# mdnunez/bayesflow_nddms

Measured on AMD Instinct MI355X. Metric: simulated DDM trials/sec at n_trials=300 dt=0.001 (basic_ddm_dc, max_steps=4000), higher is better.
Workload: dtype f32

## Files before the change

### bayesflow_nddms_amd/_lib.py

```python
import ctypes
import os

from .build import SO_PATH

NDDM_OK, NDDM_ERR_NULL, NDDM_ERR_SHAPE, NDDM_ERR_PARAM, NDDM_ERR_HIP, NDDM_ERR_NO_DEVICE = range(6)
GAUSS_EXACT, GAUSS_FAST, BRIDGE, GAUSS_PACKED, STATE_F64 = 0, 1, 2, 4, 8
QUANTILE_CONDITIONAL = 1
HMC_SIGMA_FIXED = 1
ABI_VERSION = 4

_lib = None


class NddmLibraryError(ImportError):
    pass


def _declare(L):
    c = ctypes
    fp, vp = c.c_void_p, c.c_void_p
    L.nddm_abi_version.restype = c.c_int
    L.nddm_last_error.restype = c.c_char_p
    L.nddm_device_count.argtypes = [c.POINTER(c.c_int)]
    L.nddm_set_device.argtypes = [c.c_int]
    L.nddm_summary_k.restype = c.c_int
    L.nddm_model_nparams.argtypes = [c.c_int]
    L.nddm_set_tuning.argtypes = [c.c_int] * 6
    L.nddm_set_debug_trace.argtypes = [c.c_void_p, c.c_int, c.c_int]
    L.nddm_set_ordering.argtypes = [c.c_int]
    L.nddm_debug_set_slot_limit.argtypes = [c.c_int]
    L.nddm_debug_last_launch.argtypes = [c.POINTER(c.c_int32)]
    common = [c.c_int64, c.c_int32, c.c_float, c.c_int32, c.c_uint64, c.c_uint64, c.c_uint32]
    for name in ("nddm_basic_ddm_dc_simulate", "nddm_single_trial_simulate", "nddm_single_trial_alt_simulate"):
        getattr(L, name).argtypes = [fp] + common + [fp, fp, vp]
    L.nddm_alpha_not_scaled_simulate.argtypes = [fp] + common + [c.c_float, c.c_int32, fp, fp, fp, vp]
    L.nddm_explicit_boundary_simulate.argtypes = [fp, fp] + common + [fp, fp, vp]
    L.nddm_simulratcliff.argtypes = [fp, c.c_int64, c.c_int32, c.c_uint64, c.c_uint64, c.c_uint32, c.c_float, c.c_int32, fp, fp, fp, vp]
    L.nddm_wiener_log_likelihood.argtypes = [c.c_int32, fp, c.c_int64, c.c_int64, fp, c.c_int32, c.c_uint32, fp, fp, vp]
    L.nddm_wiener_cdf.argtypes = [c.c_int32, fp, c.c_int64, c.c_int64, fp, c.c_int32, c.c_uint32, fp, fp, vp]
    L.nddm_wiener_log_likelihood_grad.argtypes = [c.c_int32, fp, c.c_int64, c.c_int64, fp, c.c_int32, c.c_uint32, fp, fp, vp]
    L.nddm_wiener_marginal_log_likelihood.argtypes = [c.c_int32, fp, c.c_int64, c.c_int64, fp, c.c_int32, c.c_float, c.c_uint32, fp, fp, vp]
    L.nddm_wiener_marginal_log_likelihood_grad.argtypes = [c.c_int32, fp, c.c_int64, c.c_int64, fp, c.c_int32, c.c_float, c.c_uint32, fp, fp, vp]
    L.nddm_wiener_hmc.argtypes = [c.c_int32, fp, c.c_int64, c.c_int32, c.c_int64, c.c_int64, fp, fp, c.c_int32, c.c_int32, c.c_int32, c.c_int32,
                                  c.c_uint32, c.c_uint64, c.c_uint64, c.c_uint64, c.c_uint32, fp, fp, fp, fp, fp, vp]
    L.nddm_wiener_hmc_joint.argtypes = [c.c_int32, fp, c.c_int64, c.c_int32, c.c_int64, c.c_int64, fp, fp, fp, fp, fp, c.c_int32, c.c_int32, c.c_int32,
                                        c.c_int32, c.c_uint32, c.c_uint64, c.c_uint64, c.c_uint64, c.c_uint32, fp, fp, fp, fp, fp, fp, fp, vp]
    L.nddm_wiener_quantile.argtypes = [c.c_int32, fp, c.c_int64, c.c_int64, fp, c.c_int32, c.c_uint32, fp, vp]
    L.nddm_simulate.argtypes = [c.c_int32, fp, fp] + common + [c.c_float, c.c_int32, fp, fp, fp, vp]
    L.nddm_simulate_indirect.argtypes = [c.c_int32, fp, fp] + common[:-1] + [fp, c.c_uint32, c.c_float, c.c_int32, fp, fp, fp, vp]
    L.nddm_simulate_codes.argtypes = [c.c_int32, fp] + common[:-1] + [fp, c.c_uint32, fp, fp, fp, vp]
    L.nddm_decode_codes.argtypes = [c.c_int32, fp, fp, c.c_int64, c.c_int32, c.c_float, fp, vp]
    L.nddm_draw_prior.argtypes = [c.c_int32, c.c_int64, c.c_uint64, c.c_uint64, c.c_float, fp, vp]
    L.nddm_draw_prior_indirect.argtypes = [c.c_int32, c.c_int64, c.c_uint64, c.c_uint64, fp, c.c_float, fp, vp]
    L.nddm_graph_arena_create.argtypes = [c.POINTER(c.c_uint64)]
    L.nddm_graph_arena_bind.argtypes = [c.c_uint64, c.POINTER(c.c_uint64)]
    L.nddm_graph_arena_info.argtypes = [c.c_uint64, c.POINTER(c.c_uint64), c.POINTER(c.c_int32)]
    L.nddm_graph_arena_release.argtypes = [c.c_uint64]
    L.nddm_source_hash.restype = c.c_char_p
    L.nddm_build_info.restype = c.c_char_p
    L.nddm_debug_normals.argtypes = [fp, c.c_int64, c.c_uint32, c.c_uint32, c.c_uint32, fp, vp]
    for name in EXPORTS:
        if name not in ("nddm_last_error", "nddm_source_hash", "nddm_build_info"):
            getattr(L, name).restype = c.c_int


EXPORTS = [
    "nddm_abi_version", "nddm_last_error", "nddm_device_count", "nddm_set_device", "nddm_summary_k",
    "nddm_model_nparams", "nddm_basic_ddm_dc_simulate", "nddm_single_trial_simulate",
    "nddm_single_trial_alt_simulate", "nddm_alpha_not_scaled_simulate", "nddm_explicit_boundary_simulate",
    "nddm_simulate", "nddm_draw_prior", "nddm_debug_normals", "nddm_set_tuning", "nddm_set_debug_trace", "nddm_set_ordering",
    "nddm_release_graph_memory", "nddm_debug_set_slot_limit", "nddm_debug_last_launch",
    "nddm_simulate_indirect", "nddm_draw_prior_indirect", "nddm_source_hash", "nddm_simulate_codes", "nddm_decode_codes",
    "nddm_graph_arena_create", "nddm_graph_arena_bind", "nddm_graph_arena_info", "nddm_graph_arena_release", "nddm_build_info",
    "nddm_simulratcliff", "nddm_wiener_log_likelihood", "nddm_wiener_cdf", "nddm_wiener_quantile",
    "nddm_wiener_log_likelihood_grad", "nddm_wiener_marginal_log_likelihood", "nddm_wiener_marginal_log_likelihood_grad",
    "nddm_wiener_hmc", "nddm_wiener_hmc_joint",
]


def lib():
    global _lib
    if _lib is None:
        from .build import build_hip, embedded_hash, is_stale, source_hash
        override = bool(os.environ.get("NDDM_HIP_LIB"))
        if is_stale():
            try:
                build_hip()
            except Exception as e:
                why = "is missing" if not os.path.exists(SO_PATH) else \
                    f"was built from other sources (library {embedded_hash()}, tree {source_hash()})"
                raise NddmLibraryError(
                    f"{SO_PATH} {why} and could not be rebuilt ({e!r}): build it with "
                    "`python -c 'import __graft_entry__ as g; g.build()'` (hipcc --offload-arch=gfx950).  "
                    "There is no CPU fallback.") from e
        if not os.path.exists(SO_PATH):
            raise NddmLibraryError(f"{SO_PATH} does not exist (NDDM_HIP_LIB points to a missing file?).  There is no CPU fallback.")
        import torch
        try:
            L = ctypes.CDLL(SO_PATH)
        except OSError as e:
            raise NddmLibraryError(f"cannot load {SO_PATH}: {e}") from e
        missing = [name for name in EXPORTS if not hasattr(L, name)]
        if missing:
            raise NddmLibraryError(f"{SO_PATH} does not export {missing}: it is older than this binding -- rebuild it "
                                   "(`python -c 'import __graft_entry__ as g; g.build()'`)")
        _declare(L)
        if L.nddm_abi_version() != ABI_VERSION:
            raise NddmLibraryError(f"ABI mismatch: library {L.nddm_abi_version()} != binding {ABI_VERSION} "
                                   "(the random stream differs between ABI versions): rebuild the library")
# ... 15 lines not shown
```

### bayesflow_nddms_amd/build.py

```python
import hashlib
import os
import re
import shutil
import subprocess

_HERE = os.path.dirname(os.path.abspath(__file__))
SO_PATH = os.environ.get("NDDM_HIP_LIB") or os.path.join(_HERE, "libnddm_hip.so")
SOURCES = [os.path.join(_HERE, "csrc", "nddm_kernels.hip")]
HEADERS = [os.path.join(_HERE, "csrc", "nddm_rng.h"), os.path.join(_HERE, "csrc", "nddm_sim.h"),
           os.path.join(_HERE, "csrc", "nddm_prepass.h"), os.path.join(_HERE, "csrc", "nddm_ratcliff.h"),
           os.path.join(_HERE, "csrc", "nddm_wiener.h"), os.path.join(_HERE, "csrc", "nddm_wiener_cdf.h"),
           os.path.join(_HERE, "csrc", "nddm_wiener_quantile.h"), os.path.join(_HERE, "csrc", "nddm_wiener_grad.h"),
           os.path.join(_HERE, "csrc", "nddm_wiener_marginal.h"), os.path.join(_HERE, "csrc", "nddm_wiener_marginal_grad.h"),
           os.path.join(_HERE, "csrc", "nddm_wiener_hmc.h"),
           os.path.join(_HERE, "csrc", "nddm_wiener_hmc_joint.h"),
           os.path.join(os.path.dirname(_HERE), "include", "nddm.h")]
HIPCC_FLAGS = ["-O3", "-ffp-contract=off", "--offload-arch=gfx950", "-fPIC", "-shared", "-std=c++17"]


def _hipcc():
    exe = shutil.which("hipcc") or "/opt/rocm/bin/hipcc"
    if not os.path.exists(exe):
        raise RuntimeError("hipcc not found: the HIP extension cannot be built")
    return exe


def source_hash():
    h = hashlib.sha256()
    for p in SOURCES + HEADERS:
        h.update(os.path.basename(p).encode() + b"\0")
        with open(p, "rb") as f:
            h.update(f.read())
        h.update(b"\0")
    h.update(" ".join(HIPCC_FLAGS).encode())
    return h.hexdigest()


def embedded_hash(path=None):
    path = path or SO_PATH
    try:
        with open(path, "rb") as f:
            m = re.search(rb"NDDM_SRC_HASH=([0-9a-f]{64})", f.read())
# ... 89 lines not shown
```

### bayesflow_nddms_amd/csrc/nddm_kernels.hip

```cpp
#include <hip/hip_runtime.h>
#include <math.h>
#include <stdint.h>
#include <stdio.h>
#include <stdlib.h>
#include <string.h>

#include <mutex>
#include <thread>

#include "../../include/nddm.h"
#include "nddm_prepass.h"
#include "nddm_ratcliff.h"
#include "nddm_rng.h"
#include "nddm_sim.h"
#include "nddm_wiener.h"
#include "nddm_wiener_cdf.h"
#include "nddm_wiener_grad.h"
#include "nddm_wiener_hmc.h"
#include "nddm_wiener_hmc_joint.h"
#include "nddm_wiener_marginal.h"
#include "nddm_wiener_marginal_grad.h"
#include "nddm_wiener_quantile.h"

namespace nddm {

static thread_local char g_err[512] = "";

static int fail(int code, const char *fmt, const char *detail = "")
{
    snprintf(g_err, sizeof g_err, fmt, detail);
    return code;
}

static int round_up_pow2(int v) { int p = 1; while (p < v) p <<= 1; return p; }

static int check_stream(hipStream_t st)
{
    int sdev = -1, cur = -1;
    const hipError_t e = hipStreamGetDevice(st, &sdev);
    if (e != hipSuccess) {
        (void)hipGetLastError();
        return fail(NDDM_ERR_HIP, "`stream` is not a live stream of this process's HIP runtime (destroyed, or created by another copy "
                                  "of the runtime): %s", hipGetErrorString(e));
    }
    if (hipGetDevice(&cur) == hipSuccess && st != nullptr && st != hipStreamPerThread && sdev != cur)
        return fail(NDDM_ERR_PARAM, "`stream` belongs to another device than the current one (nddm_set_device / hipSetDevice)%s");
    return NDDM_OK;
}

struct Tuning { int sets_per_chunk, ring, refill_thresh, variant, grid_waves, tile_trials, no_order; };
struct LastLaunch { int grid_waves, vkeys, ring, tile_trials, tiles_per_set, sets_per_chunk, refill_thresh, lds_bytes; };
static thread_local LastLaunch g_last = {0, 0, 0, 0, 0, 0, 0, 0};
static std::mutex g_mu;
static Tuning g_tuning = {0, 0, 0, 0, 0, 0, 0};
static unsigned long long *g_dbg = nullptr;
static int g_dbg_waves = 0, g_dbg_chunks = 0;

constexpr int MAX_DEVICES = 64;
struct DeviceInfo { int cus = 0; double clock_hz = 0.0; };
static DeviceInfo g_dev[MAX_DEVICES];

static bool device_info(int dev, DeviceInfo *out)
{
    std::lock_guard<std::mutex> lock(g_mu);
    if (g_dev[dev].cus == 0) {
        hipDeviceProp_t prop;
        if (hipGetDeviceProperties(&prop, dev) != hipSuccess) return false;
        g_dev[dev].cus = prop.multiProcessorCount > 0 ? prop.multiProcessorCount : 1;
        g_dev[dev].clock_hz = prop.clockRate > 0 ? (double)prop.clockRate * 1e3 : 2.4e9;
    }
    *out = g_dev[dev];
    return true;
}

constexpr size_t SLOT_QUEUE_BYTES = 256, SLOT_SCRATCH = 1u << 20;
constexpr int MAX_SLOTS = 256;
struct LaunchSlot {
    char *base = nullptr;
    hipEvent_t done = nullptr;
    hipStream_t stream = nullptr;
    bool busy = false;
    bool fresh = true;
};
static LaunchSlot *g_slots[MAX_DEVICES][MAX_SLOTS];
static int g_nslots[MAX_DEVICES];
static int g_slot_limit = MAX_SLOTS;

// ... 119 lines not shown
    *err = malloc_relaxed(&p, bytes);
    if (*err != hipSuccess) return nullptr;
    std::lock_guard<std::mutex> lock(g_mu);
    GraphArena *a = find_arena_locked(g_cur_arena);
    if (!a) a = &g_ownerless;
    a->list = new GraphAlloc{p, dev, bytes, a->list};
    return static_cast<char *>(p);
}

__global__ void zero_words_kernel(unsigned int *ws) { ws[threadIdx.x] = 0u; }

template <typename K>
static int resident_waves(K kernel, size_t lds_bytes, int cus)
{
    int per_cu = 0;
    if (hipOccupancyMaxActiveBlocksPerMultiprocessor(&per_cu, kernel, WAVE, lds_bytes) != hipSuccess || per_cu < 1)
        per_cu = 8;
    if (per_cu > 32) per_cu = 32;
    {
        const size_t granules = (lds_bytes + 1279) / 1280;
        const int by_lds = granules ? (int)((160u * 1024u) / (granules * 1280)) : 32;
        if (per_cu > by_lds) per_cu = by_lds;
    }
    hipFuncAttributes fa;
    if (hipFuncGetAttributes(&fa, reinterpret_cast<const void *>(kernel)) == hipSuccess && fa.numRegs > 0) {
        int per_simd = 512 / (((fa.numRegs + 7) / 8) * 8);
        if (per_simd < 1) per_simd = 1;
        if (per_cu > 4 * per_simd) per_cu = 4 * per_simd;
    }
    if (per_cu < 1) per_cu = 1;
    return cus * per_cu;
}

template <int MODEL, bool BRIDGE, bool SMALL, bool PACKED, bool VKEYS, bool CODES = false, bool F64 = false>
static void launch_variant(const SimArgs &A, bool fast, bool cap4, size_t lds_bytes, int n_chunks, int cus, int grid_override,
                           bool grid_forced, hipStream_t st)
{
    const dim3 block(WAVE);
#define NDDM_LAUNCH(KERNEL)                                                                    \
    do {                                                                                       \
        int waves = resident_waves(KERNEL, lds_bytes, cus);                                    \
        if (grid_override > 0 && (grid_override < waves || grid_forced)) waves = grid_override;\
        if (waves > n_chunks) waves = n_chunks;                                                \
        g_last.grid_waves = waves; g_last.vkeys = VKEYS ? 1 : 0;                               \
        hipLaunchKernelGGL(KERNEL, dim3(waves), block, lds_bytes, st, A);                      \
    } while (0)
    if (fast && cap4)       NDDM_LAUNCH((sim_kernel<MODEL, true, true, BRIDGE, SMALL, PACKED, VKEYS, CODES, F64>));
    else if (fast)          NDDM_LAUNCH((sim_kernel<MODEL, true, false, BRIDGE, SMALL, PACKED, VKEYS, CODES, F64>));
    else if (cap4)          NDDM_LAUNCH((sim_kernel<MODEL, false, true, BRIDGE, SMALL, PACKED, VKEYS, CODES, F64>));
    else                    NDDM_LAUNCH((sim_kernel<MODEL, false, false, BRIDGE, SMALL, PACKED, VKEYS, CODES, F64>));
#undef NDDM_LAUNCH
}

template <int MODEL, bool BRIDGE>
static int launch_model(const SimArgs &A, bool fast, bool packed, bool vkeys, bool f64, size_t lds_bytes, int n_chunks, int cus,
                        int grid_override, bool grid_forced, hipStream_t st)
{
    const bool cap4 = (A.max_k % ((packed || BRIDGE) ? 8 : 4)) == 0;
    const bool small = A.res16 == 2;
    constexpr bool HAS_VKEYS = !BRIDGE && (MODEL == NDDM_BASIC_DDM_DC || MODEL == NDDM_ALPHA_NOT_SCALED || MODEL == NDDM_EXPLICIT_BOUNDARY);
#define NDDM_ARGS A, fast, cap4, lds_bytes, n_chunks, cus, grid_override, grid_forced, st
    constexpr bool HAS_CODES = !BRIDGE && (MODEL == NDDM_BASIC_DDM_DC || MODEL == NDDM_ALPHA_NOT_SCALED);
    constexpr bool HAS_F64 = !BRIDGE && (MODEL == NDDM_BASIC_DDM_DC || MODEL == NDDM_SINGLE_TRIAL);
    if (f64) {
        if constexpr (HAS_F64) {
            if (small) launch_variant<MODEL, false, true, false, false, false, true>(NDDM_ARGS);
            else launch_variant<MODEL, false, false, false, false, false, true>(NDDM_ARGS);
        }
    }
    else if (A.out_codes) {
        if constexpr (HAS_CODES) launch_variant<MODEL, false, true, false, false, true>(NDDM_ARGS);
    }
    else if constexpr (BRIDGE) launch_variant<MODEL, true, false, false, false>(NDDM_ARGS);
    else if (!small && !packed) launch_variant<MODEL, false, false, false, false>(NDDM_ARGS);
    else if constexpr (HAS_VKEYS) {
        if (packed && vkeys) launch_variant<MODEL, false, true, true, true>(NDDM_ARGS);
        else if (packed) launch_variant<MODEL, false, true, true, false>(NDDM_ARGS);
        else if (vkeys) launch_variant<MODEL, false, true, false, true>(NDDM_ARGS);
        else launch_variant<MODEL, false, true, false, false>(NDDM_ARGS);
    } else {
        if (packed) launch_variant<MODEL, false, true, true, false>(NDDM_ARGS);
        else launch_variant<MODEL, false, true, false, false>(NDDM_ARGS);
    }
#undef NDDM_ARGS
    const hipError_t e = hipGetLastError();
    if (e != hipSuccess) return fail(NDDM_ERR_HIP, "kernel launch failed: %s", hipGetErrorString(e));
    return NDDM_OK;
}

static int simulate(int model, const float *params, const float *bounds, int64_t B, int32_t n_trials, float dt,
                    int32_t max_steps, uint64_t seed, uint64_t set_offset, const uint64_t *set_offset_dev, uint32_t flags,
                    float ext_sigma, int32_t ext_mode, float *out_trials, float *out_summary, float *out_ext, void *stream,
                    uint16_t *out_codes = nullptr)
{
// ... 180 lines not shown
    }
    int rc = NDDM_OK;
    A.partials = want_partials ? reinterpret_cast<unsigned long long *>(scratch + order_bytes) : nullptr;
    {
        const int threads = 256;
        long long blocks = (B + threads - 1) / threads;
        hipError_t e = hipSuccess;
        const int rec_mode = (fast ? 1 : 0) | (f64 ? 2 : 0);
        if (want_order) {
            int *order_ws = reinterpret_cast<int *>(scratch);
            uint32_t *recs = reinterpret_cast<uint32_t *>(order_ws + 64);
            if (blocks > 2048) blocks = 2048;
            hipLaunchKernelGGL(zero_words_kernel, dim3(1), dim3(64), 0, st, reinterpret_cast<unsigned int *>(order_ws));
            hipLaunchKernelGGL(order_hist_kernel, dim3((unsigned)blocks), dim3(threads), 0, st, model, params, P, (int)B, dt,
                               (int)max_steps, order_ws);
            hipLaunchKernelGGL(order_scatter_kernel, dim3((unsigned)blocks), dim3(threads), 0, st, model, rec_mode, params, P,
                               (int)B, dt, A.sqrt_dt, (int)max_steps, (unsigned long long)set_offset,
                               reinterpret_cast<const unsigned long long *>(set_offset_dev), order_ws, recs);
            A.recs = recs;
        } else {
            uint32_t *recs = reinterpret_cast<uint32_t *>(scratch);
            hipLaunchKernelGGL(prep_kernel, dim3((unsigned)blocks), dim3(threads), 0, st, model, rec_mode, params, P, (int)B, dt,
                               A.sqrt_dt, (unsigned long long)set_offset, reinterpret_cast<const unsigned long long *>(set_offset_dev), recs);
            A.recs = recs;
        }
        e = hipGetLastError();
        if (e != hipSuccess) rc = fail(NDDM_ERR_HIP, "pre-pass (hand-out records): %s", hipGetErrorString(e));
    }
    if (rc == NDDM_OK) {
        const int gw = plan_waves < 8ll * simds || tun.grid_waves > 0 ? (int)plan_waves : 0;
        bool vkeys = plan_waves < 8ll * simds || n_chunks < 8ll * simds || est_blocks < 2.0e4 * (double)simds;
        if (tun.variant % 3 == 1) vkeys = false;
        else if (tun.variant % 3 == 2) vkeys = true;
        g_last.ring = ring; g_last.tile_trials = tile_n; g_last.tiles_per_set = tiles; g_last.sets_per_chunk = spc;
        g_last.refill_thresh = A.refill_thresh; g_last.lds_bytes = (int)lds;
        switch (model) {
        case NDDM_BASIC_DDM_DC: rc = launch_model<NDDM_BASIC_DDM_DC, false>(A, fast, packed, vkeys, f64, lds, (int)n_chunks, di.cus, gw, tun.grid_waves > 0, st); break;
        case NDDM_SINGLE_TRIAL: rc = launch_model<NDDM_SINGLE_TRIAL, false>(A, fast, packed, vkeys, f64, lds, (int)n_chunks, di.cus, gw, tun.grid_waves > 0, st); break;
        case NDDM_SINGLE_TRIAL_ALT: rc = launch_model<NDDM_SINGLE_TRIAL_ALT, false>(A, fast, packed, vkeys, f64, lds, (int)n_chunks, di.cus, gw, tun.grid_waves > 0, st); break;
        case NDDM_ALPHA_NOT_SCALED:
            rc = bridge ? launch_model<NDDM_ALPHA_NOT_SCALED, true>(A, fast, packed, vkeys, f64, lds, (int)n_chunks, di.cus, gw, tun.grid_waves > 0, st)
                        : launch_model<NDDM_ALPHA_NOT_SCALED, false>(A, fast, packed, vkeys, f64, lds, (int)n_chunks, di.cus, gw, tun.grid_waves > 0, st);
            break;
        default: rc = launch_model<NDDM_EXPLICIT_BOUNDARY, false>(A, fast, packed, vkeys, f64, lds, (int)n_chunks, di.cus, gw, tun.grid_waves > 0, st); break;
        }
    }
    if (rc == NDDM_OK && A.partials) {
        const int tau_idx = model == NDDM_EXPLICIT_BOUNDARY ? 2 : 3;
        const int threads = 256;
        hipLaunchKernelGGL(combine_partials_kernel, dim3((unsigned)((B + threads - 1) / threads)), dim3(threads), 0, st,
                           A.partials, pw, params, P, tau_idx, (long long)B, tiles, n_trials, A.tscale, out_summary);
        const hipError_t e = hipGetLastError();
        if (e != hipSuccess) rc = fail(NDDM_ERR_HIP, "combine kernel launch failed: %s", hipGetErrorString(e));
    }
    if (scratch_async) (void)hipFreeAsync(scratch, st);
    if (slot) release_slot(slot, st);
    return rc;
}

struct WienerEntry {
    const char *model_msg;
    const char *flags_msg, *shape_msg, *null_in_msg, *null_out_msg;
    const char *launch_msg;
    int rows;
};

constexpr const char *WIENER_SHAPE_MSG = "R >= 0, n_trials > 0 and draws_per_dataset > 0 dividing R are required%s";
constexpr const char *WIENER_NULL_IN_MSG = "params or data is NULL%s", *WIENER_NULL_OUT_MSG = "no output buffer given%s";

static bool wiener_closed_form(int32_t model) { return model == NDDM_BASIC_DDM_DC || model == NDDM_ALPHA_NOT_SCALED; }

static int wiener_checks(const WienerEntry &E, int32_t model, bool model_ok, bool flags_ok, int64_t R, int64_t S, int32_t n, bool in_ok,
                         bool out_ok, hipStream_t st, bool *empty, bool shape_ok = true)
{
    *empty = false;
    if (!model_ok) {
        char m[16];
// ... 73 lines not shown
int nddm_summary_k(void) { return NDDM_SUMMARY_K; }

int nddm_model_nparams(int model)
{
    switch (model) {
    case NDDM_BASIC_DDM_DC: return 5;
    case NDDM_SINGLE_TRIAL: return 8;
    case NDDM_SINGLE_TRIAL_ALT: return 8;
    case NDDM_ALPHA_NOT_SCALED: return 6;
    case NDDM_EXPLICIT_BOUNDARY: return 4;
    }
    return -1;
}

int nddm_device_count(int *count)
{
    if (!count) return nddm::fail(NDDM_ERR_NULL, "count is NULL%s");
    const hipError_t e = hipGetDeviceCount(count);
    if (e != hipSuccess) { *count = 0; return nddm::fail(NDDM_ERR_NO_DEVICE, "hipGetDeviceCount: %s", hipGetErrorString(e)); }
    return NDDM_OK;
}

int nddm_set_device(int device)
{
    const hipError_t e = hipSetDevice(device);
    if (e != hipSuccess) return nddm::fail(NDDM_ERR_HIP, "hipSetDevice: %s", hipGetErrorString(e));
    return NDDM_OK;
}

int nddm_set_tuning(int sets_per_chunk, int ring, int refill_thresh, int variant, int grid_waves, int tile_trials)
{
    if (ring < 0 || ring == 1) return nddm::fail(NDDM_ERR_PARAM, "ring must be 0 (automatic) or >= 2%s");
    std::lock_guard<std::mutex> lock(nddm::g_mu);
    const int no_order = nddm::g_tuning.no_order;
    nddm::g_tuning = {sets_per_chunk, ring, refill_thresh, variant < 0 ? 0 : variant, grid_waves, tile_trials, no_order};
    return NDDM_OK;
}

int nddm_set_ordering(int enabled)
{
    std::lock_guard<std::mutex> lock(nddm::g_mu);
    nddm::g_tuning.no_order = enabled ? 0 : 1;
    return NDDM_OK;
}

int nddm_set_debug_trace(void *dev_u64, int wave_capacity, int chunk_capacity)
{
    if (dev_u64 && (wave_capacity < 0 || chunk_capacity < 0)) return nddm::fail(NDDM_ERR_PARAM, "negative trace capacity%s");
    std::lock_guard<std::mutex> lock(nddm::g_mu);
    nddm::g_dbg = static_cast<unsigned long long *>(dev_u64);
    nddm::g_dbg_waves = dev_u64 ? wave_capacity : 0;
    nddm::g_dbg_chunks = dev_u64 ? chunk_capacity : 0;
    return NDDM_OK;
}

int nddm_debug_last_launch(int32_t *out8)
{
    if (!out8) return nddm::fail(NDDM_ERR_NULL, "out8 is NULL%s");
    const nddm::LastLaunch &l = nddm::g_last;
    out8[0] = l.grid_waves; out8[1] = l.vkeys; out8[2] = l.ring; out8[3] = l.tile_trials; out8[4] = l.tiles_per_set;
    out8[5] = l.sets_per_chunk; out8[6] = l.refill_thresh; out8[7] = l.lds_bytes;
    return NDDM_OK;
}

int nddm_debug_set_slot_limit(int n)
{
    std::lock_guard<std::mutex> lock(nddm::g_mu);
    nddm::g_slot_limit = n < 1 ? 1 : (n > nddm::MAX_SLOTS ? nddm::MAX_SLOTS : n);
    return NDDM_OK;
}

int nddm_release_graph_memory(void)
{
    nddm::g_err[0] = 0;
    int dev = 0;
// ... 451 lines not shown
```

### bayesflow_nddms_amd/csrc/nddm_sim.h

```cpp
#pragma once
#include <hip/hip_runtime.h>
#include <math.h>
#include <stdint.h>

#include "../../include/nddm.h"
#include "nddm_rng.h"

namespace nddm {

constexpr int WAVE = 64;
constexpr int MAX_REJECT = 64;

typedef __attribute__((address_space(3))) uint16_t lds_u16;
typedef __attribute__((address_space(3))) uint32_t lds_u32;
typedef uint32_t u32v4 __attribute__((ext_vector_type(4)));
typedef uint32_t u32v2 __attribute__((ext_vector_type(2)));
typedef __attribute__((address_space(3))) u32v4 lds_u32v4;
typedef __attribute__((address_space(3))) u32v2 lds_u32v2;

template <int MODEL> struct ModelTraits;
template <> struct ModelTraits<NDDM_BASIC_DDM_DC>      { static constexpr int P = 5; static constexpr bool HAS_Z = false; static constexpr int TAU = 3; };
template <> struct ModelTraits<NDDM_SINGLE_TRIAL>      { static constexpr int P = 8; static constexpr bool HAS_Z = true;  static constexpr int TAU = 3; };
template <> struct ModelTraits<NDDM_SINGLE_TRIAL_ALT>  { static constexpr int P = 8; static constexpr bool HAS_Z = true;  static constexpr int TAU = 3; };
template <> struct ModelTraits<NDDM_ALPHA_NOT_SCALED>  { static constexpr int P = 6; static constexpr bool HAS_Z = false; static constexpr int TAU = 3; };
template <> struct ModelTraits<NDDM_EXPLICIT_BOUNDARY> { static constexpr int P = 4; static constexpr bool HAS_Z = true;  static constexpr int TAU = 2; };

struct SimArgs {
    const float *params;
    const float *bounds;
    float *out_trials;
    float *out_summary;
    float *out_ext;
    uint16_t *out_codes;
    long long B;
    int n_trials;
    int n_total;
    int tiles_per_set;
    unsigned long long *partials;
    const uint32_t *recs;
    int max_k;
    float dt;
    float sqrt_dt;
    float tscale;
    uint32_t k0, k1;
    int sets_per_chunk;
    int n_chunks;
    unsigned int *chunk_counter;
    int ring;
    int open_ahead;
    float ext_sigma;
    int ext_mode;
    unsigned long long *dbg;
    int dbg_waves, dbg_chunks;
    int res16;
    int refill_thresh;
    uint32_t ring_magic;
    double dt64, sqrt_dt64;
};

typedef const __attribute__((address_space(4))) SimArgs *ArgsPtr;
__device__ __forceinline__ ArgsPtr fresh_args(ArgsPtr p)
{
    asm volatile("" : "+s"(p));
    return p;
}

template <bool FAST>
struct AuxStream {
    uint32_t trial, set_lo, c3, blk, kbase;
    u32x4 x;
    __device__ __forceinline__ AuxStream(uint32_t kbase_, uint32_t set_lo_, uint32_t set_hi28, uint32_t trial_)
        : trial(trial_), set_lo(set_lo_), c3(set_hi28 | 0x10000000u), blk(0xffffffffu), kbase(kbase_) {}
    __device__ __forceinline__ void block(uint32_t b)
    {
        if (b != blk) { x = philox4x32_10_lds(set_lo, trial, c3, b, kbase); blk = b; }
    }
    __device__ __forceinline__ void first_pair(float &z0, float &z1)
    {
        block(0u);
        float r, cs, sn;
        polar_pair<FAST>(x.x, x.y, r, cs, sn);
        r *= noise_unit<FAST>(1.0f);
        z0 = r * cs; z1 = r * sn;
    }
    __device__ __forceinline__ float normal(uint32_t a)
    {
        block(a >> 2);
        const bool second = (a & 2u) != 0u;
        float r, cs, sn;
// ... 335 lines not shown
    uint32_t res_addr = 0;
    [[maybe_unused]] int tile = 0;
    bool invalid = false;
    unsigned long long has_m = 0ull, act_m = 0ull;
    constexpr int MAX_BLOCKS = 16;
    [[maybe_unused]] int cap_k = -1;
    PathCtr pc = {0u, 0u, 0u, 0u, 0u};
    [[maybe_unused]] PathKeys pkeys;
    if constexpr (VKEYS) pkeys.init(A.k0, A.k1);

    int tile_open = 0;
    int flushed = 0;
    int next_tile = 0, next_trial = 0;
    int to_retire = N;
    int chunk_set = 0, chunk_left = 0;
    int slot_pack = pack_slots(0);
    int dirty = 1;
    unsigned long long dbg_cnt = 0;
    unsigned long long *dbg_stamp = reinterpret_cast<unsigned long long *>(lds_raw + 20);
    if (lane == 0) {
        dbg_stamp[3] = 0;
        lds_raw[31] = blockIdx.x;
        if (Ak->dbg) { dbg_stamp[0] = __builtin_amdgcn_s_memtime(); dbg_stamp[1] = __builtin_amdgcn_s_memrealtime(); }
    }

    uint32_t pre = 0u;

    auto open_tiles = [&]() {
        const ArgsPtr R = fresh_args(Ak);
        while (tile_open < flushed + R->ring && tile_open <= next_tile + R->open_ahead) {
            const bool have_pre = chunk_left > 0;
            if (chunk_left <= 0) {
                if (chunk_left < 0) break;
                unsigned int c = 0;
                if (fresh_lane(lane) == 0) c = atomicAdd(R->chunk_counter, 1u);
                c = __builtin_amdgcn_readfirstlane(c);
                if (c >= (unsigned int)R->n_chunks) {
                    chunk_left = -1;
                    if (fresh_lane(lane) == 0 && R->dbg) dbg_stamp[3] = __builtin_amdgcn_s_memrealtime();
                    break;
                }
                if (fresh_lane(lane) == 0 && R->dbg && c < (unsigned int)R->dbg_chunks)
                    R->dbg[8ll * R->dbg_waves + c] = __builtin_amdgcn_s_memrealtime();
                chunk_set = (int)c * R->sets_per_chunk;
                const long long left = R->B - (long long)chunk_set;
                chunk_left = (int)(left < R->sets_per_chunk ? left : R->sets_per_chunk);
            }
            const int slot = ring_slot(tile_open, R->ring, R->ring_magic);
            const int TPS = R->tiles_per_set;
            const int prow = TPS == 1 ? chunk_set : chunk_set / TPS;
            const int qt = chunk_set - prow * TPS;
            uint32_t rec = pre;
            if (!have_pre) rec = fresh_lane(lane) < REC ? R->recs[(long long)prow * REC + lane] : 0u;
            if (chunk_left > 1) {
                const int nrow = TPS == 1 ? chunk_set + 1 : (chunk_set + 1) / TPS;
                if (nrow != prow) pre = fresh_lane(lane) < REC ? R->recs[(long long)nrow * REC + lane] : 0u;
                else pre = rec;
            }
            const int sic = __builtin_amdgcn_readlane((int)rec, R_SET);
            const int vset = sic * TPS + qt;
            uint32_t *d = slot_rec(slot);
            if (lane < REC) d[lane] = rec;
            const uint32_t s_lo = (uint32_t)__builtin_amdgcn_readlane((int)rec, R_GLO);
            const uint32_t s_hi = (uint32_t)__builtin_amdgcn_readlane((int)rec, R_GHI);
            if (lane == 0) {
                d[D_VSET] = (uint32_t)vset;
                if constexpr (MODEL == NDDM_SINGLE_TRIAL || MODEL == NDDM_SINGLE_TRIAL_ALT) { d[D_ZSUM] = 0u; d[D_ZSUM + 1] = 0u; d[D_ZSUM + 2] = 0u; d[D_ZSUM + 3] = 0u; }
                PathSet ps;
                ps.init(s_lo, s_hi, R->k0, R->k1);
                d[D_CA] = ps.cA; d[D_CB] = ps.cB; d[D_HP1K] = ps.hP1k; d[D_X1] = ps.X1;
// ... 312 lines not shown
                             "v_cmp_gt_i32 vcc, %[ck], %[k]\n\t"
                             "s_and_b64 %[am], %[am], vcc\n"
                             "2:"
                             : [w] "+v"(w), [k] "+v"(k), [am] "+s"(act_m)
                             : [ck] "s"(cap_k), [mu] "v"(mu_dt), [h] "v"(h), [r0] "v"(rr[0]), [r1] "v"(rr[2]),
                               [t0] "v"(tt[0]), [t1] "v"(tt[1]), [t2] "v"(tt[2]), [t3] "v"(tt[3])
                             : "vcc", "scc");
#undef NDDM_STEP
#undef NDDM_K2
                if ((int)__popcll(has_m & ~act_m) >= leave_at) break;
                if (it >= it_limit) break;
                continue;
            }
#pragma unroll
            for (int j = 0; j < NS; ++j) {
                if (active) {
                    asm volatile("" ::: "memory");
                    w = __builtin_fmaf(rr[j], tt[j], w) + mu_dt;
                    k++;
                    if (j < NS - 1) {
                        if constexpr (CAP4) active = in_range(w, h);
                        else active = in_range(w, h) && (k < A.max_k);
                    }
                }
            }
            act_m = __builtin_amdgcn_ballot_w64(in_range(w, h)) & __builtin_amdgcn_ballot_w64(k < A.max_k) & has_m;
            if ((int)__popcll(has_m & ~act_m) >= leave_at) break;
            if (it >= it_limit) break;
        }
        dbg_cnt += (1ull << 32) | (unsigned long long)(uint32_t)(it + 1);
    }
    if (lane == 0) {
        unsigned int *const q = fresh_args(Ak)->chunk_counter;
        const unsigned int left = atomicAdd(q + 1, 1u);
        if (left == gridDim.x - 1u) { atomicExch(q, 0u); atomicExch(q + 1, 0u); }
    }
    unsigned long long *const dbg = fresh_args(Ak)->dbg;
    if (dbg && lane == 0) {
        const unsigned long long t_end = __builtin_amdgcn_s_memrealtime(), c_end = __builtin_amdgcn_s_memtime();
        const uint32_t wg = lds_raw[31];
        if (wg < (uint32_t)fresh_args(Ak)->dbg_waves) {
            unsigned long long *const r = dbg + 8ull * wg;
            r[0] = dbg_cnt & 0xffffffffull; r[1] = dbg_cnt >> 32;
            r[2] = c_end - dbg_stamp[0]; r[3] = t_end - dbg_stamp[1];
            r[4] = dbg_stamp[1]; r[5] = dbg_stamp[3]; r[6] = t_end; r[7] = 1ull;
        }
    }
}

}
```

### include/nddm.h

```cpp
#ifndef NDDM_H
#define NDDM_H

#include <stdint.h>

#ifdef __cplusplus
extern "C" {
#endif

#define NDDM_ABI_VERSION 4
#define NDDM_SUMMARY_K 10

enum nddm_summary_col {
    NDDM_S_N_UPPER = 0,
    NDDM_S_N_LOWER = 1,
    NDDM_S_N_MISSING = 2,
    NDDM_S_MEAN_RT = 3,
    NDDM_S_VAR_RT = 4,
    NDDM_S_MEAN_RT_UPPER = 5,
    NDDM_S_VAR_RT_UPPER = 6,
    NDDM_S_MEAN_Z = 7,
    NDDM_S_VAR_Z = 8,
    NDDM_S_CHOICE_MEAN = 9
};

// ... 7 lines not shown

enum nddm_status {
    NDDM_OK = 0,
    NDDM_ERR_NULL = 1,
    NDDM_ERR_SHAPE = 2,
    NDDM_ERR_PARAM = 3,
    NDDM_ERR_HIP = 4,
    NDDM_ERR_NO_DEVICE = 5
};

enum nddm_flags {
    NDDM_GAUSS_EXACT = 0,
    NDDM_GAUSS_FAST = 1,
    NDDM_GAUSS_PACKED = 4,
    NDDM_STATE_F64 = 8,
    NDDM_BRIDGE = 2
};

int nddm_abi_version(void);
const char *nddm_last_error(void);
int nddm_device_count(int *count);
int nddm_set_device(int device);
int nddm_summary_k(void);
int nddm_model_nparams(int model);
int nddm_graph_arena_create(uint64_t *arena);
int nddm_graph_arena_bind(uint64_t arena, uint64_t *previous );
int nddm_graph_arena_info(uint64_t arena, uint64_t *bytes , int32_t *n_allocations );
int nddm_graph_arena_release(uint64_t arena);
int nddm_release_graph_memory(void);
int nddm_debug_set_slot_limit(int n);
int nddm_debug_last_launch(int32_t *out8);
int nddm_set_tuning(int sets_per_chunk, int ring, int refill_thresh, int variant, int grid_waves, int tile_trials);
int nddm_set_ordering(int enabled);
int nddm_set_debug_trace(void *dev_u64, int wave_capacity, int chunk_capacity);


int nddm_basic_ddm_dc_simulate(const float *params, int64_t B, int32_t n_trials, float dt, int32_t max_steps,
                               uint64_t seed, uint64_t set_offset, uint32_t flags, float *out_trials,
                               float *out_summary, void *stream);

int nddm_single_trial_simulate(const float *params, int64_t B, int32_t n_trials, float dt, int32_t max_steps,
                               uint64_t seed, uint64_t set_offset, uint32_t flags, float *out_trials,
                               float *out_summary, void *stream);

int nddm_single_trial_alt_simulate(const float *params, int64_t B, int32_t n_trials, float dt, int32_t max_steps,
                                   uint64_t seed, uint64_t set_offset, uint32_t flags, float *out_trials,
                                   float *out_summary, void *stream);

int nddm_alpha_not_scaled_simulate(const float *params, int64_t B, int32_t n_trials, float dt, int32_t max_steps,
                                   uint64_t seed, uint64_t set_offset, uint32_t flags, float ext_sigma,
                                   int32_t ext_mode, float *out_trials, float *out_summary, float *out_extdata,
                                   void *stream);

int nddm_simulratcliff(const float *params, int64_t B, int32_t n_trials, uint64_t seed, uint64_t set_offset, uint32_t flags,
                       float ext_sigma, int32_t ext_mode, float *out_trials, float *out_summary, float *out_extdata, void *stream);

int nddm_wiener_log_likelihood(int32_t model, const float *params, int64_t R, int64_t draws_per_dataset, const float *data,
                               int32_t n_trials, uint32_t flags, float *out_trial_logp ,
                               double *out_loglik , void *stream);

int nddm_wiener_log_likelihood_grad(int32_t model, const float *params, int64_t R, int64_t draws_per_dataset, const float *data,
                                    int32_t n_trials, uint32_t flags , double *out_loglik ,
                                    double *out_grad , void *stream);

int nddm_wiener_hmc(int32_t model, const float *data , int64_t D, int32_t n_trials, int64_t C,
                    int64_t chains_per_dataset, double *state , const double *inv_mass , int32_t n_iter,
// ... 67 lines not shown
```

Before: 9.573 billion.

## Split chunk work queue into front and back ends for dynamic load balancing

Replaces the single atomic chunk counter with a packed 64-bit front/back counter, so a subset of waves (about 3/8 by default when ordering is on and chunks are plentiful) pulls chunks from the tail of the queue while the rest pull from the head. The aim is to balance uneven per-chunk work, presumably because ordered chunks vary in cost from one end to the other, and to reduce tail imbalance. It changes the counter layout (the done-counter moves to offset 2) and adds a tuning entry point. It risks changing chunk assignment and the tail behaviour.

```diff
diff --git a/bayesflow_nddms_amd/_lib.py b/bayesflow_nddms_amd/_lib.py
--- a/bayesflow_nddms_amd/_lib.py
+++ b/bayesflow_nddms_amd/_lib.py
@@ -28,6 +28,7 @@
     L.nddm_set_tuning.argtypes = [c.c_int] * 6
     L.nddm_set_debug_trace.argtypes = [c.c_void_p, c.c_int, c.c_int]
     L.nddm_set_ordering.argtypes = [c.c_int]
+    L.nddm_set_queue_split.argtypes = [c.c_int]
     L.nddm_debug_set_slot_limit.argtypes = [c.c_int]
     L.nddm_debug_last_launch.argtypes = [c.POINTER(c.c_int32)]
     common = [c.c_int64, c.c_int32, c.c_float, c.c_int32, c.c_uint64, c.c_uint64, c.c_uint32]
@@ -74,7 +75,7 @@
     "nddm_graph_arena_create", "nddm_graph_arena_bind", "nddm_graph_arena_info", "nddm_graph_arena_release", "nddm_build_info",
     "nddm_simulratcliff", "nddm_wiener_log_likelihood", "nddm_wiener_cdf", "nddm_wiener_quantile",
     "nddm_wiener_log_likelihood_grad", "nddm_wiener_marginal_log_likelihood", "nddm_wiener_marginal_log_likelihood_grad",
-    "nddm_wiener_hmc", "nddm_wiener_hmc_joint",
+    "nddm_wiener_hmc", "nddm_wiener_hmc_joint", "nddm_set_queue_split",
 ]
 
 
diff --git a/bayesflow_nddms_amd/build.py b/bayesflow_nddms_amd/build.py
--- a/bayesflow_nddms_amd/build.py
+++ b/bayesflow_nddms_amd/build.py
@@ -7,7 +7,7 @@
 _HERE = os.path.dirname(os.path.abspath(__file__))
 SO_PATH = os.environ.get("NDDM_HIP_LIB") or os.path.join(_HERE, "libnddm_hip.so")
 SOURCES = [os.path.join(_HERE, "csrc", "nddm_kernels.hip")]
-HEADERS = [os.path.join(_HERE, "csrc", "nddm_rng.h"), os.path.join(_HERE, "csrc", "nddm_sim.h"),
+HEADERS = [os.path.join(_HERE, "csrc", "nddm_rng.h"), os.path.join(_HERE, "csrc", "nddm_sim.h"), os.path.join(_HERE, "csrc", "nddm_queue.h"),
            os.path.join(_HERE, "csrc", "nddm_prepass.h"), os.path.join(_HERE, "csrc", "nddm_ratcliff.h"),
            os.path.join(_HERE, "csrc", "nddm_wiener.h"), os.path.join(_HERE, "csrc", "nddm_wiener_cdf.h"),
            os.path.join(_HERE, "csrc", "nddm_wiener_quantile.h"), os.path.join(_HERE, "csrc", "nddm_wiener_grad.h"),
diff --git a/bayesflow_nddms_amd/csrc/nddm_kernels.hip b/bayesflow_nddms_amd/csrc/nddm_kernels.hip
--- a/bayesflow_nddms_amd/csrc/nddm_kernels.hip
+++ b/bayesflow_nddms_amd/csrc/nddm_kernels.hip
@@ -48,11 +48,11 @@
     return NDDM_OK;
 }
 
-struct Tuning { int sets_per_chunk, ring, refill_thresh, variant, grid_waves, tile_trials, no_order; };
+struct Tuning { int sets_per_chunk, ring, refill_thresh, variant, grid_waves, tile_trials, no_order, queue_split; };
 struct LastLaunch { int grid_waves, vkeys, ring, tile_trials, tiles_per_set, sets_per_chunk, refill_thresh, lds_bytes; };
 static thread_local LastLaunch g_last = {0, 0, 0, 0, 0, 0, 0, 0};
 static std::mutex g_mu;
-static Tuning g_tuning = {0, 0, 0, 0, 0, 0, 0};
+static Tuning g_tuning = {0, 0, 0, 0, 0, 0, 0, -1};
 static unsigned long long *g_dbg = nullptr;
 static int g_dbg_waves = 0, g_dbg_chunks = 0;
 
@@ -238,17 +238,28 @@
     return cus * per_cu;
 }
 
+constexpr int QUEUE_SPLIT_AUTO = -1, QUEUE_SPLIT_OFF = 0;
+constexpr int QUEUE_SPLIT_NUM = 3, QUEUE_SPLIT_DEN = 8, QUEUE_SPLIT_MIN_CHUNKS = 12;
+static int back_waves(int queue_split, int waves, int n_chunks, bool vkeys)
+{
+    if (queue_split > 0) return queue_split < waves ? queue_split : waves;
+    if (queue_split != QUEUE_SPLIT_AUTO || vkeys || (long long)n_chunks < (long long)QUEUE_SPLIT_MIN_CHUNKS * waves) return 0;
+    return (int)((long long)waves * QUEUE_SPLIT_NUM / QUEUE_SPLIT_DEN);
+}
+
 template <int MODEL, bool BRIDGE, bool SMALL, bool PACKED, bool VKEYS, bool CODES = false, bool F64 = false>
-static void launch_variant(const SimArgs &A, bool fast, bool cap4, size_t lds_bytes, int n_chunks, int cus, int grid_override,
-                           bool grid_forced, hipStream_t st)
+static void launch_variant(const SimArgs &A0, bool fast, bool cap4, size_t lds_bytes, int n_chunks, int cus, int grid_override,
+                           bool grid_forced, int queue_split, hipStream_t st)
 {
     const dim3 block(WAVE);
+    SimArgs A = A0;
 #define NDDM_LAUNCH(KERNEL)                                                                    \
     do {                                                                                       \
         int waves = resident_waves(KERNEL, lds_bytes, cus);                                    \
         if (grid_override > 0 && (grid_override < waves || grid_forced)) waves = grid_override;\
         if (waves > n_chunks) waves = n_chunks;                                                \
         g_last.grid_waves = waves; g_last.vkeys = VKEYS ? 1 : 0;                               \
+        A.back_from = waves - back_waves(queue_split, waves, n_chunks, VKEYS);                 \
         hipLaunchKernelGGL(KERNEL, dim3(waves), block, lds_bytes, st, A);                      \
     } while (0)
     if (fast && cap4)       NDDM_LAUNCH((sim_kernel<MODEL, true, true, BRIDGE, SMALL, PACKED, VKEYS, CODES, F64>));
@@ -260,12 +271,12 @@
 
 template <int MODEL, bool BRIDGE>
 static int launch_model(const SimArgs &A, bool fast, bool packed, bool vkeys, bool f64, size_t lds_bytes, int n_chunks, int cus,
-                        int grid_override, bool grid_forced, hipStream_t st)
+                        int grid_override, bool grid_forced, int queue_split, hipStream_t st)
 {
     const bool cap4 = (A.max_k % ((packed || BRIDGE) ? 8 : 4)) == 0;
     const bool small = A.res16 == 2;
     constexpr bool HAS_VKEYS = !BRIDGE && (MODEL == NDDM_BASIC_DDM_DC || MODEL == NDDM_ALPHA_NOT_SCALED || MODEL == NDDM_EXPLICIT_BOUNDARY);
-#define NDDM_ARGS A, fast, cap4, lds_bytes, n_chunks, cus, grid_override, grid_forced, st
+#define NDDM_ARGS A, fast, cap4, lds_bytes, n_chunks, cus, grid_override, grid_forced, queue_split, st
     constexpr bool HAS_CODES = !BRIDGE && (MODEL == NDDM_BASIC_DDM_DC || MODEL == NDDM_ALPHA_NOT_SCALED);
     constexpr bool HAS_F64 = !BRIDGE && (MODEL == NDDM_BASIC_DDM_DC || MODEL == NDDM_SINGLE_TRIAL);
     if (f64) {
@@ -512,17 +523,18 @@
         bool vkeys = plan_waves < 8ll * simds || n_chunks < 8ll * simds || est_blocks < 2.0e4 * (double)simds;
         if (tun.variant % 3 == 1) vkeys = false;
         else if (tun.variant % 3 == 2) vkeys = true;
+        const int qsplit = tun.queue_split >= 0 ? tun.queue_split : (want_order && gw == 0 ? QUEUE_SPLIT_AUTO : QUEUE_SPLIT_OFF);
         g_last.ring = ring; g_last.tile_trials = tile_n; g_last.tiles_per_set = tiles; g_last.sets_per_chunk = spc;
         g_last.refill_thresh = A.refill_thresh; g_last.lds_bytes = (int)lds;
         switch (model) {
-        case NDDM_BASIC_DDM_DC: rc = launch_model<NDDM_BASIC_DDM_DC, false>(A, fast, packed, vkeys, f64, lds, (int)n_chunks, di.cus, gw, tun.grid_waves > 0, st); break;
-        case NDDM_SINGLE_TRIAL: rc = launch_model<NDDM_SINGLE_TRIAL, false>(A, fast, packed, vkeys, f64, lds, (int)n_chunks, di.cus, gw, tun.grid_waves > 0, st); break;
-        case NDDM_SINGLE_TRIAL_ALT: rc = launch_model<NDDM_SINGLE_TRIAL_ALT, false>(A, fast, packed, vkeys, f64, lds, (int)n_chunks, di.cus, gw, tun.grid_waves > 0, st); break;
+        case NDDM_BASIC_DDM_DC: rc = launch_model<NDDM_BASIC_DDM_DC, false>(A, fast, packed, vkeys, f64, lds, (int)n_chunks, di.cus, gw, tun.grid_waves > 0, qsplit, st); break;
+        case NDDM_SINGLE_TRIAL: rc = launch_model<NDDM_SINGLE_TRIAL, false>(A, fast, packed, vkeys, f64, lds, (int)n_chunks, di.cus, gw, tun.grid_waves > 0, qsplit, st); break;
+        case NDDM_SINGLE_TRIAL_ALT: rc = launch_model<NDDM_SINGLE_TRIAL_ALT, false>(A, fast, packed, vkeys, f64, lds, (int)n_chunks, di.cus, gw, tun.grid_waves > 0, qsplit, st); break;
         case NDDM_ALPHA_NOT_SCALED:
-            rc = bridge ? launch_model<NDDM_ALPHA_NOT_SCALED, true>(A, fast, packed, vkeys, f64, lds, (int)n_chunks, di.cus, gw, tun.grid_waves > 0, st)
-                        : launch_model<NDDM_ALPHA_NOT_SCALED, false>(A, fast, packed, vkeys, f64, lds, (int)n_chunks, di.cus, gw, tun.grid_waves > 0, st);
+            rc = bridge ? launch_model<NDDM_ALPHA_NOT_SCALED, true>(A, fast, packed, vkeys, f64, lds, (int)n_chunks, di.cus, gw, tun.grid_waves > 0, qsplit, st)
+                        : launch_model<NDDM_ALPHA_NOT_SCALED, false>(A, fast, packed, vkeys, f64, lds, (int)n_chunks, di.cus, gw, tun.grid_waves > 0, qsplit, st);
             break;
-        default: rc = launch_model<NDDM_EXPLICIT_BOUNDARY, false>(A, fast, packed, vkeys, f64, lds, (int)n_chunks, di.cus, gw, tun.grid_waves > 0, st); break;
+        default: rc = launch_model<NDDM_EXPLICIT_BOUNDARY, false>(A, fast, packed, vkeys, f64, lds, (int)n_chunks, di.cus, gw, tun.grid_waves > 0, qsplit, st); break;
         }
     }
     if (rc == NDDM_OK && A.partials) {
@@ -662,8 +674,8 @@
 {
     if (ring < 0 || ring == 1) return nddm::fail(NDDM_ERR_PARAM, "ring must be 0 (automatic) or >= 2%s");
     std::lock_guard<std::mutex> lock(nddm::g_mu);
-    const int no_order = nddm::g_tuning.no_order;
-    nddm::g_tuning = {sets_per_chunk, ring, refill_thresh, variant < 0 ? 0 : variant, grid_waves, tile_trials, no_order};
+    const int no_order = nddm::g_tuning.no_order, queue_split = nddm::g_tuning.queue_split;
+    nddm::g_tuning = {sets_per_chunk, ring, refill_thresh, variant < 0 ? 0 : variant, grid_waves, tile_trials, no_order, queue_split};
     return NDDM_OK;
 }
 
@@ -671,6 +683,13 @@
 {
     std::lock_guard<std::mutex> lock(nddm::g_mu);
     nddm::g_tuning.no_order = enabled ? 0 : 1;
+    return NDDM_OK;
+}
+
+int nddm_set_queue_split(int back_waves)
+{
+    std::lock_guard<std::mutex> lock(nddm::g_mu);
+    nddm::g_tuning.queue_split = back_waves < 0 ? -1 : back_waves;
     return NDDM_OK;
 }
 
diff --git a/bayesflow_nddms_amd/csrc/nddm_queue.h b/bayesflow_nddms_amd/csrc/nddm_queue.h
--- /dev/null
+++ b/bayesflow_nddms_amd/csrc/nddm_queue.h
@@ -0,0 +1,15 @@
+#pragma once
+#include <hip/hip_runtime.h>
+#include <stdint.h>
+
+namespace nddm {
+
+constexpr unsigned long long QUEUE_FRONT = 1ull, QUEUE_BACK = 1ull << 32;
+__host__ __device__ inline long long queue_pull(unsigned long long old, int n_chunks, bool back)
+{
+    const unsigned long long f = old & 0xffffffffull, b = old >> 32;
+    if (f + b >= (unsigned long long)(long long)n_chunks) return -1;
+    return back ? (long long)n_chunks - 1 - (long long)b : (long long)f;
+}
+
+}
diff --git a/bayesflow_nddms_amd/csrc/nddm_sim.h b/bayesflow_nddms_amd/csrc/nddm_sim.h
--- a/bayesflow_nddms_amd/csrc/nddm_sim.h
+++ b/bayesflow_nddms_amd/csrc/nddm_sim.h
@@ -4,6 +4,7 @@
 #include <stdint.h>
 
 #include "../../include/nddm.h"
+#include "nddm_queue.h"
 #include "nddm_rng.h"
 
 namespace nddm {
@@ -55,6 +56,7 @@
     int res16;
     int refill_thresh;
     uint32_t ring_magic;
+    int back_from;
     double dt64, sqrt_dt64;
 };
 
@@ -456,10 +458,15 @@
             const bool have_pre = chunk_left > 0;
             if (chunk_left <= 0) {
                 if (chunk_left < 0) break;
-                unsigned int c = 0;
-                if (fresh_lane(lane) == 0) c = atomicAdd(R->chunk_counter, 1u);
-                c = __builtin_amdgcn_readfirstlane(c);
-                if (c >= (unsigned int)R->n_chunks) {
+                const bool from_back = __builtin_amdgcn_readfirstlane((int)lds_raw[31]) >= R->back_from;
+                unsigned long long old = 0ull;
+                if (fresh_lane(lane) == 0)
+                    old = atomicAdd(reinterpret_cast<unsigned long long *>(R->chunk_counter), from_back ? QUEUE_BACK : QUEUE_FRONT);
+                old = ((unsigned long long)(uint32_t)__builtin_amdgcn_readfirstlane((int)(old >> 32)) << 32) |
+                      (uint32_t)__builtin_amdgcn_readfirstlane((int)(uint32_t)old);
+                const long long pulled = queue_pull(old, R->n_chunks, from_back);
+                const unsigned int c = (unsigned int)pulled;
+                if (pulled < 0) {
                     chunk_left = -1;
                     if (fresh_lane(lane) == 0 && R->dbg) dbg_stamp[3] = __builtin_amdgcn_s_memrealtime();
                     break;
@@ -838,8 +845,8 @@
     }
     if (lane == 0) {
         unsigned int *const q = fresh_args(Ak)->chunk_counter;
-        const unsigned int left = atomicAdd(q + 1, 1u);
-        if (left == gridDim.x - 1u) { atomicExch(q, 0u); atomicExch(q + 1, 0u); }
+        const unsigned int left = atomicAdd(q + 2, 1u);
+        if (left == gridDim.x - 1u) { atomicExch(reinterpret_cast<unsigned long long *>(q), 0ull); atomicExch(q + 2, 0u); }
     }
     unsigned long long *const dbg = fresh_args(Ak)->dbg;
     if (dbg && lane == 0) {
diff --git a/include/nddm.h b/include/nddm.h
--- a/include/nddm.h
+++ b/include/nddm.h
@@ -63,6 +63,7 @@
 int nddm_debug_last_launch(int32_t *out8);
 int nddm_set_tuning(int sets_per_chunk, int ring, int refill_thresh, int variant, int grid_waves, int tile_trials);
 int nddm_set_ordering(int enabled);
+int nddm_set_queue_split(int back_waves);
 int nddm_set_debug_trace(void *dev_u64, int wave_capacity, int chunk_capacity);
 
 
```

Result: faster. 9.673 billion (median of 6 runs) (+1.0%).
